# vpariza/open-hummingbird-eval

Measured on AMD Instinct MI355X. Metric: query-patches/sec, higher is better.
Workload: dtype f32

## Files before the change

### include/hbird_hip.h

```cpp
#ifndef HBIRD_HIP_H
#define HBIRD_HIP_H
#include <stdint.h>
#ifdef __cplusplus
extern "C" {
#endif

typedef struct hb_index hb_index_t;

#define HB_METRIC_IP 0
#define HB_METRIC_L2 1
#define HB_MAX_K 2048
#define HB_MAX_K_AGGREGATE 256
#define HB_BIGK_MAX_PARTS 64

const char* hb_last_error(void);
int hb_device_count(int* n);

int hb_index_create(int d, int metric, int device, hb_index_t** out);
int hb_index_free(hb_index_t* ix);
int hb_index_set_stream(hb_index_t* ix, void* hip_stream);
int hb_index_reserve(hb_index_t* ix, int64_t n_rows);
int hb_index_add(hb_index_t* ix, const float* x, int64_t n, int x_on_device, int normalize);
int hb_index_add_labels(hb_index_t* ix, const float* labels, int64_t n, int c, int on_device);
int hb_index_set_label_denominator(hb_index_t* ix, int P);
// ... 110 lines not shown
int hb_schedule_plan_weighted(int nqt, int nbt, int workgroups, int panel_tiles, int d, int cluster_q, int cluster_b, int shared,
                              const double* xcd_w8, int* segs_out, int64_t max_segs, int64_t stats[8]);
int hb_index_wg_stamps(hb_index_t* ix, uint32_t* out, int max_blocks, int* workgroups);
int hb_index_kernel_clock(hb_index_t* ix, double out[4]);
int hb_index_xcd_stats(const hb_index_t* ix, int fp16_kernel, double out[12]);
int hb_debug_live_allocations(int64_t* count, int64_t* bytes);
void* hb_calibration_new(int fp16_kernel);
void hb_calibration_free(void* h);
int hb_calibration_state(const void* h, double shares8[8], int64_t out[12]);
int hb_calibration_feed(void* h, const uint32_t* stamps, int G, const double run_shares8[8], const int key6[6], int auto_cluster, double frac);
int hb_f16_adapt_replay(int n, const double* f1, const double* f2, int64_t nq, int* out_how);
int hb_set_layout_form(int form);
int hb_index_set_rerank_copy(hb_index_t* ix, int mode);
int hb_index_rerank_copy_bytes(const hb_index_t* ix, int64_t* bytes);
int hb_index_schedule_info(const hb_index_t* ix, int64_t out[8]);
int hb_index_set_cluster(hb_index_t* ix, int cluster_q, int cluster_b, int sync_lag);
int hb_index_set_cluster_sharing(hb_index_t* ix, int mode);
int hb_index_cluster_stats(hb_index_t* ix, int64_t out[4]);

int hb_schedule_plan(int nqt, int nbt, int workgroups, int panel_tiles, int d, int cluster_q, int cluster_b, int* segs_out,
                     int64_t max_segs, int64_t stats[8]);
int hb_schedule_plan_phased(int nqt, int nbt, int workgroups, int panel_tiles, int d, int cluster_q, int cluster_b, int* segs_out,
                            int64_t max_segs, int64_t stats[8], int* clocks_out, int max_cuts, int* n_cuts, int* bounds_out);

int hb_schedule_plan_shared(int nqt, int nbt, int workgroups, int panel_tiles, int d, int cluster_q, int cluster_b, int phased,
                            int* segs_out, int64_t max_segs, int64_t stats[8]);

#include "hbird_hip_centre.h"
#include "hbird_hip_select.h"
#include "hbird_hip_grid.h"
#include "hbird_hip_exclude.h"
#include "hbird_hip_screen.h"
#include "hbird_hip_exclude_screen.h"
#include "hbird_hip_kmeans.h"
#include "hbird_hip_linprobe.h"
#include "hbird_hip_depth.h"

#ifdef __cplusplus
}
#endif
#endif
// ... 1 lines not shown
```

### open-hummingbird-eval_amd/csrc/hbird_calibrate.cpp

```cpp
#include "hbird_calibrate.h"
#include "hbird_certificate.h"
#include <algorithm>
#include <cmath>
#include <vector>

bool hb_stamps_summarise(const unsigned* st, int G, hb_stamp_summary& o) {
    if (G < 8 || G % 8 != 0) return false;
    std::vector<double> dur[8], every, ghz;
    const unsigned s0 = st[0];
    long long first = 0, last = 0;
    for (int b = 0; b < G; ++b) {
        const unsigned* sb = st + 8 * (size_t)b;
        const unsigned t0 = sb[0], t1 = sb[4], xcc = sb[1];
        if (t0 == 0u && t1 == 0u) return false;
        if (xcc > 7u || sb[5] != xcc) return false;
        if (b < 8) o.xcc[b] = (int)xcc;
        else if ((int)xcc != o.xcc[b & 7]) return false;
        const unsigned d = t1 - t0;
        if (d == 0u || d > 0x7FFFFFFFu) return false;
        dur[b & 7].push_back((double)d); every.push_back((double)d);
        const long long rs = (long long)(int)(t0 - s0), re = rs + (long long)d;
        if (b == 0) { first = rs; last = re; }
        first = std::min(first, rs); last = std::max(last, re);
        const unsigned long long c0 = ((unsigned long long)sb[3] << 32) | sb[2], c1 = ((unsigned long long)sb[7] << 32) | sb[6];
// ... 156 lines not shown
    if (in.ceil) { cq = 1; cb = 1; }
    else if (in.force_cq > 0 && in.force_cb > 0) { cq = in.force_cq; cb = in.force_cb; }
    else if (f16 && in.variant == 0 && in.force_cq == 0) {
        if (hb_stages_per_wg(nqt, nbt, G, in.dp16 / 16) >= 70000) hb_default_cluster(nqt, nbt, G, false, &cq, &cb);
    }
    else if (!f16 && !p.wide && in.variant == 0 && in.force_cq == 0 && in.g8 % 4 == 0 && hb_stages_per_wg(nqt, nbt, G, in.g8) >= 1000000) {
        p.auto_cluster = true;
        const bool measured = in.xcd_balance == 0 && G % 8 == 0;
        if (in.cl_state == 2 ? in.cl_choice != 0 : (!measured || in.cl_state == 0)) hb_default_cluster(nqt, nbt, G, true, &cq, &cb);
    }
    if ((long long)nqt * nbt < G || cq * cb > HB_CLUSTER_MAX || G % (8 * cq * cb) != 0) { cq = 1; cb = 1; }
    p.cq = cq; p.cb = cb;
    const size_t tile_bytes = (size_t)HB_BT * in.dp * 4;
    p.panel = in.force_panel > 0 ? in.force_panel : hb_default_panel(nqt, std::min<long long>(G, (long long)nqt * nbt), tile_bytes, cq, cb);
    p.phased = p.wide && in.phases_on && in.esc == 0;
    p.xs = cq * cb > 1 && (in.xcd_share == 2 || (in.xcd_share == 0 && f16));
    p.lag = cq * cb > 1 ? (in.sync_lag >= 0 ? in.sync_lag : 16) : 0;
}

void hb_knn_plan_kernel(const hb_knn_plan_in& in, int sched_G, hb_knn_plan& p) {
    const bool clustered = p.cq * p.cb > 1;
    const long long stages_per_wg = hb_stages_per_wg(p.nqt, p.nbt, sched_G, in.g8);
    p.small = !in.f16 && !clustered && stages_per_wg < (in.k > HB_KL ? std::min<long long>(p.small_limit, 50000) : p.small_limit);
    if (in.f16) p.kernel = HB_KERNEL_F16;
    else if (in.ceil) p.kernel = HB_KERNEL_CEIL;
    else if (p.bd_shape && (in.variant == 0 || in.variant == 3 || in.variant == 6)) p.kernel = HB_KERNEL_BD + (p.wide ? 4 : 0) + (clustered ? 2 : 0) + (p.small ? 1 : 0);
    else if (clustered) p.kernel = p.wide ? HB_KERNEL_POOLS_CL : HB_KERNEL_LISTS_CL;
    else if (p.small && !p.wide) p.kernel = HB_KERNEL_LISTS_COLD;
    else p.kernel = p.wide ? HB_KERNEL_POOLS : HB_KERNEL_LISTS;
}

struct hb_calibration { hb_xcd_state st; int fam; };
// ... 51 lines not shown
    hb_knn_plan_in pin;
    pin.f16 = in[0] != 0; pin.wide_first = in[1] != 0; pin.esc = (int)in[2]; pin.ceil = in[3] != 0;
    pin.k = (int)in[4]; pin.nq = in[5]; pin.ntotal = in[6]; pin.g8 = (int)in[7]; pin.dp = (int)in[8]; pin.dp16 = (int)in[9]; pin.num_cu = (int)in[10];
    pin.force_G = (int)in[11]; pin.force_panel = (int)in[12]; pin.force_cq = (int)in[13]; pin.force_cb = (int)in[14]; pin.variant = (int)in[15];
    pin.small_limit = in[16]; pin.phases_on = (int)in[17]; pin.xcd_balance = (int)in[18]; pin.xcd_share = (int)in[19]; pin.sync_lag = (int)in[20];
    pin.cl_state = (int)in[21]; pin.cl_choice = (int)in[22];
    hb_knn_plan p;
    hb_knn_plan_shape(pin, p);
    hb_knn_plan_clusters(pin, p);
    const long long pairs = (long long)p.nqt * p.nbt;
    const int sched_G = n_in > 23 && in[23] > 0 ? (int)in[23] : pairs < p.G ? (int)std::max<long long>(1, pairs) : p.G;
    hb_knn_plan_kernel(pin, sched_G, p);
    out[0] = p.kc; out[1] = p.wide; out[2] = p.klw; out[3] = p.small_pools; out[4] = p.nqt; out[5] = p.nbt; out[6] = p.G; out[7] = p.fam; out[8] = p.balance;
    out[9] = p.cq; out[10] = p.cb; out[11] = p.auto_cluster; out[12] = p.panel; out[13] = p.phased; out[14] = p.xs; out[15] = p.lag; out[16] = p.kernel;
    out[17] = sched_G; out[18] = p.small;
    return 0;
}
extern "C" int hb_certificate_bound_replay(const double* in, int n_in, double* out, int n_out) {
    if (!in || !out || n_in < 8 || n_out < 2 || !(in[0] >= 1.0 && in[0] <= 1048576.0)) return -1;
    const int d = (int)in[0], metric = in[1] != 0.0 ? 1 : 0;
    const float qn = (float)in[2], bmax = (float)in[3], qc = (float)in[4], cmax = (float)in[5], mun = (float)in[6], at = fabsf((float)in[7]);
    out[0] = (double)hb_certificate_bound(qn, bmax, d, metric);
    out[1] = (double)hb_certificate_bound_centred(qc, cmax, mun, at, qn, bmax, d, metric);
    return 0;
}
int hb_exclude_plan(int k, int64_t gmax, int rungs[2]) {
    if (k < 1 || k > HB_MAX_K || gmax < 0) return -1;
    const int64_t need = (int64_t)k + gmax;
    if (need > HB_MAX_K) return -2;
    const int64_t r0 = 256 * (((int64_t)k + std::min<int64_t>(k, gmax) + 255) / 256);
// ... 18 lines not shown
```

### open-hummingbird-eval_amd/csrc/hbird_calibrate.h

```cpp
#pragma once
#include <array>
#include <stdint.h>
#include "../../include/hbird_hip.h"
#include "hbird_schedule.h"

#define HB_POOL_MAX 512
#define HB_KL 32

struct hb_stamp_summary {
    double med[8];
    int xcc[8];
    double all;
    double span_ticks;
    double ghz_med, ghz_min, ghz_max;
};
bool hb_stamps_summarise(const unsigned* st, int G, hb_stamp_summary& o);

struct hb_xcd_state {
    double w[8] = {1, 1, 1, 1, 1, 1, 1, 1};
    int rounds = 0;
    int samples = 0, rejected = 0;
    std::array<int, 6> key{{0, 0, 0, 0, 0, 0}};
    double cur_w[8] = {1, 1, 1, 1, 1, 1, 1, 1}, best_w[8] = {1, 1, 1, 1, 1, 1, 1, 1};
    double cur_span = 0.0, best_span = 0.0;
// ... 53 lines not shown
    int phases_on = 1, xcd_balance = 0, xcd_share = 0, sync_lag = -1;
    int cl_state = 0, cl_choice = 1;
};
enum hb_knn_kernel {
    HB_KERNEL_F16 = 0,
    HB_KERNEL_LISTS = 1, HB_KERNEL_LISTS_COLD = 2, HB_KERNEL_POOLS = 3, HB_KERNEL_LISTS_CL = 4, HB_KERNEL_POOLS_CL = 5, HB_KERNEL_CEIL = 6,
    HB_KERNEL_BD = 8
};
struct hb_knn_plan {
    int kc = 0; bool wide = false; int klw = 0; bool small_pools = false;
    int nqt = 0, nbt = 0, G = 0, fam = 0; bool balance = false;
    bool calibrated = false;
    long long small_limit = 0; bool bd_shape = false;
    int cq = 1, cb = 1; bool auto_cluster = false; int panel = 0;
    bool phased = false, xs = false; int lag = 0;
    bool small = false; int kernel = HB_KERNEL_LISTS;
};
long long hb_stages_per_wg(long long nqt, long long nbt, int workgroups, int stages_per_tile);
long long hb_stages_per_busy_wg(long long nqt, long long nbt, int workgroups, int stages_per_tile);
inline int hb_knn_workgroups(int force_G, int num_cu) { return force_G > 0 ? force_G : num_cu; }
void hb_knn_plan_shape(const hb_knn_plan_in& in, hb_knn_plan& p);
void hb_knn_plan_clusters(const hb_knn_plan_in& in, hb_knn_plan& p);
void hb_knn_plan_kernel(const hb_knn_plan_in& in, int sched_G, hb_knn_plan& p);

int hb_exclude_plan(int k, int64_t gmax, int rungs[2]);
```

### open-hummingbird-eval_amd/csrc/hbird_capi.hip

```cpp
#include "../../include/hbird_hip.h"
#include "hbird_internal.h"
#include <algorithm>
#include <atomic>
#include <cmath>
#include <cstdlib>
#include <cstring>
#include <dlfcn.h>
#include <mutex>
#include <set>
#include <utility>

static thread_local std::string g_err;
void hb_set_error(const std::string& msg) { g_err = msg; }
int hb_fail(const std::string& msg) { g_err = msg; return -1; }

static std::atomic<int64_t> g_live_allocs{0}, g_live_bytes{0};
const char* hb_dev_alloc(void** p, size_t bytes) {
    const hipError_t e = hipMalloc(p, bytes);
    if (e != hipSuccess) { (void)hipGetLastError(); *p = nullptr; return hipGetErrorString(e); }
    ++g_live_allocs; g_live_bytes += (int64_t)bytes;
    return nullptr;
}
void hb_dev_free(void* p, size_t bytes) {
    (void)hipFree(p);
// ... 166 lines not shown
}
extern "C" int hb_index_last_fp16_escalated(const hb_index_t* ix, int64_t* n) {
    if (!ix || !n) return hb_fail("hb_index_last_fp16_escalated: NULL pointer");
    *n = ix->last.escalated;
    return 0;
}
extern "C" int hb_index_last_fp16_fallbacks(const hb_index_t* ix, int64_t* n) {
    if (!ix || !n) return hb_fail("hb_index_last_fp16_fallbacks: NULL pointer");
    *n = ix->last.fallbacks;
    return 0;
}


extern "C" int hb_index_set_cluster_sharing(hb_index_t* ix, int mode) {
    if (!ix) return hb_fail("hb_index_set_cluster_sharing: NULL index handle");
    if (mode < 0 || mode > 2) return hb_fail("hb_index_set_cluster_sharing: mode must be 0 (automatic), 1 (off) or 2 (on)");
    ix->xcd_share = mode; ix->sched = hb_schedule(); ix->fp32_pinned = 1;
    return 0;
}

extern "C" int hb_index_cluster_stats(hb_index_t* ix, int64_t out[4]) {
    if (!ix || !out) return hb_fail("hb_index_cluster_stats: NULL pointer");
    out[0] = out[1] = out[2] = out[3] = 0;
    if (!ix->cl_stats_dev) return 0;
    HB_HIP(hipSetDevice(ix->device));
    int h[4] = {0, 0, 0, 0};
    HB_HIP(hipMemcpyAsync(h, ix->cl_stats_dev, sizeof(h), hipMemcpyDeviceToHost, ix->stream));
    HB_HIP(hipStreamSynchronize(ix->stream));
    out[0] = h[0]; out[1] = h[1]; out[2] = h[2]; out[3] = h[3];
    return 0;
}
// ... 106 lines not shown
    }
    return 0;
}
extern "C" int hb_index_rerank_copy_bytes(const hb_index_t* ix, int64_t* bytes) {
    if (!ix || !bytes) return hb_fail("hb_index_rerank_copy_bytes: NULL argument");
    *bytes = ix->row_copy.bytes();
    return 0;
}
extern "C" int hb_index_schedule_info(const hb_index_t* ix, int64_t out[8]) {
    if (!ix) return hb_fail("hb_index_schedule_info: NULL index handle");
    const hb_schedule& s = ix->sched;
    out[0] = s.G; out[1] = (int64_t)s.segs.size(); out[2] = s.n_slots; out[3] = s.panel; out[4] = s.max_slots_per_qt;
    out[5] = s.nqt; out[6] = s.nbt; out[7] = s.cq * 16 + s.cb;
    return 0;
}

int hb_index::bank_changed(hb_bank_event what) {
    last.bank_changed();
    if (what == HB_BANK_EMPTIED) {
        copy16.emptied(); row_copy.m.emptied();
        if (copy16.flag) HB_HIP(hipMemsetAsync(copy16.flag, 0, 4, stream));
    }
    return 0;
}

extern "C" int hb_index_reserve(hb_index_t* ix, int64_t n_rows) {
    if (!ix) return hb_fail("hb_index_reserve: NULL index handle");
    HB_HIP(hipSetDevice(ix->device));
    int64_t cap = (n_rows + HB_BT - 1) / HB_BT * HB_BT;
    if (cap <= ix->cap_rows) return 0;
// ... 409 lines not shown
```

### open-hummingbird-eval_amd/csrc/hbird_knn.hip

```cpp
#include "hbird_internal.h"
#include "../../include/hbird_hip.h"
#include <algorithm>
#include <array>
#include <mutex>
#include <cstring>
#include <map>

#include "hbird_knn_dev.h"
#include "hbird_rerank_dev.h"

#define KN_MFMA(T, FR, B, S) acc[T] = __builtin_amdgcn_mfma_f32_32x32x2f32(FR[(T) & 3][S], B[S], acc[T], 0, 0, 0);

template <bool COLD, bool WIDE, bool CL = false, bool CEIL = false>
__global__ __launch_bounds__(HB_THREADS, 2) void knn_fused_kernel(knn_args a) {
    extern __shared__ __attribute__((aligned(16))) char smem[];
    const int tid = threadIdx.x;
    const int lane = tid & 63;
    const int w = __builtin_amdgcn_readfirstlane(tid >> 6);
    const int h = lane >> 5;
    float* lst_s = reinterpret_cast<float*>(smem + KN_LISTS);
    unsigned* lst_i = reinterpret_cast<unsigned*>(smem + KN_LISTS + HB_QT * HB_KL * 4);
    float* sc = reinterpret_cast<float*>(smem + KN_SCRATCH) + w * 256;
    unsigned* qf = reinterpret_cast<unsigned*>(smem + KN_QF) + w * 512;
    int* pcnt = reinterpret_cast<int*>(smem + KN_LISTS);
// ... 596 lines not shown
    knn_work_list& wl = *out;
    static const double equal_shares[8] = {1, 1, 1, 1, 1, 1, 1, 1};
    if (p.balance) {
        double shares_n[8];
        double mean = 0.0;
        bool uneven = false;
        const hb_index::xcd_cal& xc = ix->xcal[p.fam];
        for (int x = 0; x < 8; ++x) mean += xc.w[x] / 8.0;
        for (int g = 0; g < 8; ++g) { shares_n[g] = xc.w[ix->xcd_balance == 0 ? xc.perm[g] : g] / mean; uneven = uneven || std::fabs(shares_n[g] - 1.0) > 1e-9; }
        if (uneven) std::copy(shares_n, shares_n + 8, wl.shares);
    }
    const double* shares = wl.shares;
    hb_schedule& sc = esc == 0 ? ix->sched : ix->sched_esc;
    hb_dev<char>& sched_dev = esc == 0 ? ix->sched_dev : ix->sched_esc_dev;
    const int nqt = p.nqt, nbt = p.nbt, G = p.G;
    const bool rebuilt = !(sc.nqt == nqt && sc.nbt == nbt && sc.panel == p.panel && sc.cq == p.cq && sc.cb == p.cb && sc.phased == p.phased &&
                           sc.xcd_share == p.xs && (sc.G == G || (long long)nqt * nbt < G) &&
                           (sc.xcd_w.empty() ? std::equal(shares, shares + 8, equal_shares) : std::equal(shares, shares + 8, sc.xcd_w.begin())));
    if (rebuilt) { hb_build_schedule(nqt, nbt, G, p.panel, sc, p.cq, p.cb, p.phased, p.xs, shares); ++ix->sched_builds; }
    const struct { const void* data; size_t bytes; } part[6] = {{sc.segs.data(), sc.segs.size() * sizeof(hb_seg)}, {sc.wg_off.data(), sc.wg_off.size() * 4},
        {sc.qt_off.data(), sc.qt_off.size() * 4}, {sc.qt_slots.data(), sc.qt_slots.size() * 4}, {sc.wg_member.data(), sc.wg_member.size() * 4},
        {sc.phase_bounds.data(), sc.phase_bounds.size() * 4}};
    size_t off[7] = {0};
    for (int i = 0; i < 6; ++i) off[i + 1] = off[i] + al256(part[i].bytes);
    const bool need_upload = rebuilt || sched_dev.bytes < off[6];
    if (sched_dev.ensure(off[6], HB_GROW_QUARTER)) return -1;
    if (need_upload) {
        for (int i = 0; i < 6; ++i) HB_HIP(hipMemcpyAsync(sched_dev + off[i], part[i].data, part[i].bytes, hipMemcpyHostToDevice, s));
        HB_HIP(hipStreamSynchronize(s));
    }
    auto ints = [&](int i) { return sched_dev.as<const int>(off[i]); };
    wl.sc = &sc; wl.segs = sched_dev.as<const hb_seg>();
    wl.wg_off = ints(1); wl.qt_off = ints(2); wl.qt_slots = ints(3); wl.wg_member = ints(4); wl.phase_bounds = ints(5);
    wl.n_phases = (int)sc.phase_clock.size() + 1;
// ... 326 lines not shown
```

### open-hummingbird-eval_amd/csrc/hbird_schedule.cpp

```cpp
#include "hbird_schedule.h"
#include <algorithm>
#include <cmath>
#include <map>

#ifdef HB_PLAN_STANDALONE
static thread_local std::string g_plan_err;
int hb_fail(const std::string& msg) { g_plan_err = msg; return -1; }
extern "C" const char* hb_last_error(void) { return g_plan_err.c_str(); }
#endif

static int hb_gcd(int x, int y) { while (y) { int t = x % y; x = y; y = t; } return x; }

int hb_default_panel(int nqt, int G, size_t tile_bytes, int cq, int cb) {
    int p0;
    if (cq * cb > 1) {
        const int NC = std::max(1, G / (cq * cb)), NQG = (nqt + cq - 1) / cq;
        p0 = cb * (NC / hb_gcd(NQG, NC));
    } else p0 = G / hb_gcd(nqt, G);
    size_t budget = (size_t)96 << 20;
    int j = (int)std::max<size_t>(1, budget / (tile_bytes * (size_t)p0));
    return p0 * j;
}

void hb_default_cluster(int nqt, int nbt, int G, bool fp32_kernel, int* cq, int* cb) {
// ... 82 lines not shown
}

static std::vector<double> hb_cum_shares(int workers, int per_xcd, const std::vector<double>& xcd_w) {
    std::vector<double> cum(workers + 1, 0.0);
    for (int i = 0; i < workers; ++i) cum[i + 1] = cum[i] + xcd_w[std::min(7, i / std::max(1, per_xcd))];
    for (int i = 0; i <= workers; ++i) cum[i] /= cum[workers];
    return cum;
}
static long long hb_share_bound(long long W, const std::vector<double>& cum, int i, int workers, int panel_index) {
    if (i <= 0) return 0;
    if (i >= workers) return W;
    const double phi = std::fmod(0.5 + 0.6180339887498949 * panel_index, 1.0);
    return std::min<long long>(W, std::max<long long>(0, (long long)std::floor((double)W * cum[i] + phi)));
}

static void hb_build_clustered(int nqt, int nbt, int G, int panel, int cq, int cb, hb_schedule& out, bool xcd_share) {
    const int CS = cq * cb, NC = G / CS, NQG = (nqt + cq - 1) / cq;
    out.cq = cq; out.cb = cb; out.n_clusters = NC; out.xcd_share = xcd_share;
    std::vector<std::vector<hb_seg>> per_wg(G);
    std::vector<int> slot_of((size_t)G * nqt, -1);
    std::vector<std::vector<int>> slots_of_qt(nqt);
    std::vector<int> clock(NC, 0);
    auto deal = [&](int c, int b0, int pp, int qg, int j0, int cnt) {
        for (int m = 0; m < CS; ++m) {
            const int ia = m / cb, ib = m % cb, q = qg * cq + ia, w = c * CS + m;
            int n = cnt;
            if ((j0 + cnt - 1) * cb + ib >= pp) --n;
            if (q >= nqt || n <= 0) continue;
            hb_seg sg;
            sg.q_tile = q; sg.b_tile0 = b0 + j0 * cb + ib; sg.n_tiles = n; sg.stride = cb; sg.tile0 = clock[c]; sg.next_tile0 = 0;
            int& known = slot_of[(size_t)w * nqt + q];
            if (known < 0) {
                sg.slot = out.n_slots++; sg.first = 1;
                known = sg.slot;
                slots_of_qt[q].push_back(sg.slot);
            } else { sg.slot = known; sg.first = 0; }
            per_wg[w].push_back(sg);
        }
        clock[c] += cnt;
    };
    const int per_xcd_c = NC / 8;
    int rot = 0;
    const std::vector<double> cum = (!out.xcd_w.empty() && !xcd_share && NC % 8 == 0) ? hb_cum_shares(NC, NC / 8, out.xcd_w) : std::vector<double>();
    const std::vector<double> cumx = (!out.xcd_w.empty() && xcd_share) ? hb_cum_shares(8, 1, out.xcd_w) : std::vector<double>();
    for (int b0 = 0; b0 < nbt; b0 += panel) {
        const int pp = std::min(panel, nbt - b0);
        const int UB = (pp + cb - 1) / cb;
        const long long U = (long long)NQG * UB;
        if (xcd_share) {
            for (int x = 0; x < 8; ++x) {
                long long e = (U * x) / 8;
                long long e1 = (U * (x + 1)) / 8;
                if (!cumx.empty()) { e = hb_share_bound(U, cumx, x, 8, b0 / panel); e1 = hb_share_bound(U, cumx, x + 1, 8, b0 / panel); }
                while (e < e1) {
                    const int qg = (int)(e / UB), j0 = (int)(e % UB);
                    const int L = (int)std::min<long long>(UB - j0, e1 - e);
                    for (int i = 0; i < per_xcd_c; ++i) {
                        const int a0 = (int)((long long)L * i / per_xcd_c), a1 = (int)((long long)L * (i + 1) / per_xcd_c);
                        if (a1 > a0) deal(x * per_xcd_c + (i + rot) % per_xcd_c, b0, pp, qg, j0 + a0, a1 - a0);
                    }
                    ++rot;
                    e += L;
                }
            }
            continue;
        }
        for (int c = 0; c < NC; ++c) {
            long long e0 = (U * c) / NC, e1 = (U * (c + 1)) / NC;
            if (!cum.empty()) { e0 = hb_share_bound(U, cum, c, NC, b0 / panel); e1 = hb_share_bound(U, cum, c + 1, NC, b0 / panel); }
            while (e0 < e1) {
                const int qg = (int)(e0 / UB), j0 = (int)(e0 % UB);
                const int cnt = (int)std::min<long long>(UB - j0, e1 - e0);
                deal(c, b0, pp, qg, j0, cnt);
                e0 += cnt;
            }
        }
    }
    std::vector<int> logical_of_block(G);
    out.wg_member.assign(G, -1);
    const int per_xcd = NC / 8;
    for (int c = 0; c < NC; ++c)
        for (int m = 0; m < CS; ++m) {
            const int block = c / per_xcd + 8 * ((c % per_xcd) * CS + m);
            logical_of_block[block] = c * CS + m;
            out.wg_member[block] = c * HB_CLUSTER_LINE + m;
        }
    hb_finish_schedule(out, per_wg, logical_of_block, slots_of_qt);
}

void hb_build_schedule(int nqt, int nbt, int G, int panel, hb_schedule& out, int cq, int cb, bool phased, bool xcd_share, const double* xcd_w) {
    out = hb_schedule();
    out.nqt = nqt; out.nbt = nbt; out.panel = panel; out.phased = phased;
    if (xcd_w) {
        bool ok = true, equal = true;
        for (int x = 0; x < 8; ++x) { ok = ok && xcd_w[x] > 0.25 && xcd_w[x] < 4.0; equal = equal && xcd_w[x] == xcd_w[0]; }
        if (ok && !equal) out.xcd_w.assign(xcd_w, xcd_w + 8);
    }
    const long long total_pairs = (long long)nqt * nbt;
    if (total_pairs < G) G = (int)std::max<long long>(1, total_pairs);
    out.G = G;
    if (phased) {
        const long long per_wg_tiles = total_pairs / G;
        long long t = 0, step = 1;
        while (out.phase_clock.size() < HB_PHASE_CUTS) {
            t += step;
            if (t * 2 > per_wg_tiles) break;
            out.phase_clock.push_back((int)t);
            step = std::max<long long>(step + 1, per_wg_tiles <= 64 ? step * 3 : step < 128 ? step * 3 / 2 : step * 2);
        }
    }
    if (cq < 1 || cb < 1 || cq * cb > HB_CLUSTER_MAX || G % (8 * cq * cb) != 0) { cq = 1; cb = 1; }
    if (cq * cb > 1) { hb_build_clustered(nqt, nbt, G, panel, cq, cb, out, xcd_share); return; }
    std::vector<std::vector<hb_seg>> per_wg(G);
    std::vector<int> slot_of((size_t)G * nqt, -1);
    std::vector<std::vector<int>> slots_of_qt(nqt);
    std::vector<int> clock(G, 0);
    const std::vector<double> cum = (!out.xcd_w.empty() && G % 8 == 0) ? hb_cum_shares(G, G / 8, out.xcd_w) : std::vector<double>();
    for (int b0 = 0; b0 < nbt; b0 += panel) {
        const int pp = std::min(panel, nbt - b0);
        const long long W = (long long)nqt * pp;
        for (int w = 0; w < G; ++w) {
            long long e0 = (W * w) / G, e1 = (W * (w + 1)) / G;
            if (!cum.empty()) { e0 = hb_share_bound(W, cum, w, G, b0 / panel); e1 = hb_share_bound(W, cum, w + 1, G, b0 / panel); }
            while (e0 < e1) {
                const int q = (int)(e0 / pp), b = (int)(e0 % pp);
                const int cnt = (int)std::min<long long>(pp - b, e1 - e0);
                int& known = slot_of[(size_t)w * nqt + q];
// ... 16 lines not shown
    }
    std::vector<int> logical_of_block(G);
    for (int b = 0; b < G; ++b) {
        if (G % 8 == 0) logical_of_block[b] = (b % 8) * (G / 8) + b / 8;
        else {
            const int q = G / 8, r = G % 8, x = b % 8;
            logical_of_block[b] = (x < r ? x * (q + 1) : r * (q + 1) + (x - r) * q) + b / 8;
        }
    }
    out.wg_member.assign(G, -1);
    hb_finish_schedule(out, per_wg, logical_of_block, slots_of_qt);
}


static int schedule_plan(int nqt, int nbt, int workgroups, int panel_tiles, int d, int cluster_q, int cluster_b, bool phased,
                         int* segs_out, int64_t max_segs, int64_t stats[8], hb_schedule& sc, bool xcd_share = false, const double* xcd_w = nullptr) {
    if (!stats) return hb_fail("hb_schedule_plan: stats is NULL");
    if (nqt <= 0 || nbt <= 0 || workgroups <= 0 || d <= 0) return hb_fail("hb_schedule_plan: bad arguments");
    const int dp = (d + HB_KC - 1) / HB_KC * HB_KC;
    const int G = (int)std::min<long long>(workgroups, (long long)nqt * nbt);
    int cq = cluster_q, cb = cluster_b;
    if (cq < 0 || cb < 0) hb_default_cluster(nqt, nbt, G, cq == -2, &cq, &cb);
    if (cq < 1 || cb < 1 || (long long)nqt * nbt < workgroups || cq * cb > HB_CLUSTER_MAX || G % (8 * cq * cb) != 0) { cq = 1; cb = 1; }
    const int panel = panel_tiles > 0 ? panel_tiles : hb_default_panel(nqt, G, (size_t)HB_BT * dp * 4, cq, cb);
    hb_build_schedule(nqt, nbt, workgroups, panel, sc, cq, cb, phased, xcd_share && cq * cb > 1, xcd_w);
    stats[0] = sc.G; stats[1] = (int64_t)sc.segs.size(); stats[2] = sc.n_slots; stats[3] = sc.panel;
    stats[4] = sc.max_slots_per_qt; stats[5] = sc.nqt; stats[6] = sc.nbt; stats[7] = sc.cq * 16 + sc.cb;
    if (segs_out) {
        int64_t n = 0;
        for (int b = 0; b < sc.G; ++b)
            for (int i = sc.wg_off[b]; i < sc.wg_off[b + 1] && n < max_segs; ++i, ++n) {
                const hb_seg& g = sc.segs[i];
                int* o = segs_out + n * 10;
                o[0] = b; o[1] = g.q_tile; o[2] = g.b_tile0; o[3] = g.n_tiles; o[4] = g.slot; o[5] = g.first;
                o[6] = g.stride; o[7] = g.tile0; o[8] = g.next_tile0; o[9] = sc.wg_member[b];
            }
    }
    return 0;
}

// ... 17 lines not shown
    }
    return 0;
}

extern "C" int hb_schedule_plan_weighted(int nqt, int nbt, int workgroups, int panel_tiles, int d, int cluster_q, int cluster_b, int shared,
                                         const double* xcd_w8, int* segs_out, int64_t max_segs, int64_t stats[8]) {
    hb_schedule sc;
    return schedule_plan(nqt, nbt, workgroups, panel_tiles, d, cluster_q, cluster_b, (shared & 2) != 0, segs_out, max_segs, stats, sc, (shared & 1) != 0, xcd_w8);
}

extern "C" int hb_schedule_plan_shared(int nqt, int nbt, int workgroups, int panel_tiles, int d, int cluster_q, int cluster_b, int phased,
                                       int* segs_out, int64_t max_segs, int64_t stats[8]) {
    hb_schedule sc;
    return schedule_plan(nqt, nbt, workgroups, panel_tiles, d, cluster_q, cluster_b, phased != 0, segs_out, max_segs, stats, sc, true);
}
```

### open-hummingbird-eval_amd/csrc/hbird_schedule.h

```cpp
#pragma once
#include <stddef.h>
#include <stdint.h>
#include <string>
#include <vector>

#define HB_QT 256
#define HB_BT 256
#define HB_KC 16

struct hb_seg {
    int q_tile;
    int b_tile0;
    int n_tiles;
    int slot;
    int first;
    int stride;
    int tile0;
    int next_tile0;
    int ord;
    int nsl;
};

#define HB_PHASE_CUTS 24
#define HB_CLUSTER_MAX 8
// ... 4 lines not shown
    int cq = 1, cb = 1;
    bool xcd_share = false;
    std::vector<double> xcd_w;
    std::vector<hb_seg> segs;
    std::vector<int> wg_off;
    std::vector<int> wg_member;
    bool phased = false;
    std::vector<int> phase_clock;
    bool cuts_scaled = false;
    std::vector<int> phase_bounds;
    std::vector<int> qt_off;
    std::vector<int> qt_slots;
    int n_slots = 0;
    int max_slots_per_qt = 0;
    int n_clusters = 0;
};

void hb_build_schedule(int nqt, int nbt, int G, int panel_tiles, hb_schedule& out, int cq = 1, int cb = 1, bool phased = false,
                       bool xcd_share = false, const double* xcd_w = nullptr);
int hb_default_panel(int nqt, int G, size_t tile_bytes, int cq = 1, int cb = 1);
void hb_default_cluster(int nqt, int nbt, int G, bool fp32_kernel, int* cq, int* cb);

int hb_fail(const std::string& msg);
```

### open-hummingbird-eval_amd/hbird_mi/_lib.py

```python
from __future__ import annotations

import ctypes
import os
from ctypes import POINTER, c_char_p, c_double, c_float, c_int, c_int32, c_int64, c_uint64, c_void_p

_PKG_ROOT = os.path.dirname(os.path.dirname(os.path.abspath(__file__)))
LIB_PATH = os.environ.get("HBIRD_HIP_LIB") or os.path.join(_PKG_ROOT, "lib", "libhbird_hip.so")
CSRC_DIR = os.path.join(_PKG_ROOT, "csrc")

_lib = None

SIGNATURES = {
    "hb_last_error": (c_char_p, []),
    "hb_device_count": (c_int, [POINTER(c_int)]),
    "hb_index_create": (c_int, [c_int, c_int, c_int, POINTER(c_void_p)]),
    "hb_index_free": (c_int, [c_void_p]),
    "hb_index_set_stream": (c_int, [c_void_p, c_void_p]),
    "hb_index_reserve": (c_int, [c_void_p, c_int64]),
    "hb_index_add": (c_int, [c_void_p, c_void_p, c_int64, c_int, c_int]),
    "hb_index_add_labels": (c_int, [c_void_p, c_void_p, c_int64, c_int, c_int]),
    "hb_index_ntotal": (c_int64, [c_void_p]),
    "hb_index_nlabels": (c_int64, [c_void_p]),
    "hb_index_reset": (c_int, [c_void_p]),
    "hb_index_search": (c_int, [c_void_p, c_void_p, c_int64, c_int, c_int64, c_void_p, c_void_p, c_int]),
# ... 41 lines not shown
                                       c_void_p]),
    "hb_argmax_channels": (c_int, [c_void_p, c_int64, c_int, c_void_p, c_void_p]),
    "hb_confusion_update": (c_int, [c_void_p, c_void_p, c_int64, c_int, c_int, c_int64, c_int, c_void_p, c_void_p]),
    "hb_index_set_timing": (c_int, [c_void_p, c_int]),
    "hb_index_last_knn_ms": (c_int, [c_void_p, POINTER(c_double)]),
    "hb_index_set_tuning": (c_int, [c_void_p, c_int, c_int]),
    "hb_index_set_fp16": (c_int, [c_void_p, c_int]),
    "hb_index_last_fp16_fallbacks": (c_int, [c_void_p, POINTER(c_int64)]),
    "hb_last_search_path": (c_int, [c_void_p, POINTER(c_int), POINTER(c_int)]),
    "hb_index_set_fp16_escalation": (c_int, [c_void_p, c_int]),
    "hb_index_last_fp16_escalated": (c_int, [c_void_p, POINTER(c_int64)]),
    "hb_schedule_plan": (c_int, [c_int, c_int, c_int, c_int, c_int, c_int, c_int, c_void_p, c_int64, POINTER(c_int64)]),
    "hb_schedule_plan_phased": (c_int, [c_int, c_int, c_int, c_int, c_int, c_int, c_int, c_void_p, c_int64, POINTER(c_int64),
                                        c_void_p, c_int, POINTER(c_int), c_void_p]),
    "hb_schedule_plan_shared": (c_int, [c_int, c_int, c_int, c_int, c_int, c_int, c_int, c_int, c_void_p, c_int64, POINTER(c_int64)]),
    "hb_index_set_cluster": (c_int, [c_void_p, c_int, c_int, c_int]),
    "hb_index_set_cluster_sharing": (c_int, [c_void_p, c_int]),
    "hb_index_set_label_denominator": (c_int, [c_void_p, c_int]),
    "hb_index_labels_to_fp32": (c_int, [c_void_p]),
    "hb_index_label_denominator": (c_int, [c_void_p, POINTER(c_int)]),
    "hb_index_copy_label_counts": (c_int, [c_void_p, c_void_p, c_int]),
    "hb_index_set_label_count_table": (c_int, [c_void_p, c_void_p, c_void_p, c_int64, c_int, c_int, c_int64]),
    "hb_index_cluster_stats": (c_int, [c_void_p, POINTER(c_int64)]),
    "hb_index_set_variant": (c_int, [c_void_p, c_int]),
    "hb_index_set_search_options": (c_int, [c_void_p, c_int, c_int64]),
    "hb_index_wg_stamps": (c_int, [c_void_p, c_void_p, c_int, POINTER(c_int)]),
    "hb_index_set_xcd_weights": (c_int, [c_void_p, c_int, POINTER(c_double)]),
    "hb_index_xcd_weights": (c_int, [c_void_p, c_int, POINTER(c_double), POINTER(c_int)]),
    "hb_schedule_plan_weighted": (c_int, [c_int, c_int, c_int, c_int, c_int, c_int, c_int, c_int, POINTER(c_double), c_void_p, c_int64, POINTER(c_int64)]),
    "hb_index_kernel_clock": (c_int, [c_void_p, POINTER(c_double)]),
# ... 172 lines not shown
```

### open-hummingbird-eval_amd/hbird_mi/nn/search_hip.py

```python
from __future__ import annotations

import ctypes
import math
from collections import namedtuple
from typing import Optional, Tuple

import numpy as np
import torch

from hbird_mi import _lib
from hbird_mi.nn.search_base import NearestNeighborSearchBase

_METRICS = {"dot_product": 0, "l2": 1, "euclidean": 1}
MAX_K = 256
MAX_K_SEARCH = 2048
_MERGE_LDS = 60000


def k5(index, name: str, k: int):
    return getattr(index, name + "_bigk" if k > MAX_K and hasattr(index, name + "_bigk") else name)


def check_k(k: int, what: str = "k"):
    if not 1 <= k <= MAX_K_SEARCH:
# ... 615 lines not shown

    def set_cluster_sharing(self, mode: int = 0):
        _lib.check(_lib.lib().hb_index_set_cluster_sharing(self._h, int(mode)))

    def cluster_stats(self) -> dict:
        out = (ctypes.c_int64 * 4)()
        _lib.check(_lib.lib().hb_index_cluster_stats(self._h, out))
        return {"checks": int(out[0]), "waits": int(out[1]), "timeouts": int(out[2])}

    def schedule_info(self) -> dict:
        out = (ctypes.c_int64 * 8)()
        _lib.check(_lib.lib().hb_index_schedule_info(self._h, out))
        keys = ["workgroups", "segments", "slots", "panel_tiles", "max_slots_per_qtile", "query_tiles", "bank_tiles"]
        d = dict(zip(keys, list(out)[:7]))
        d["cluster"] = [int(out[7]) // 16, int(out[7]) % 16]
        return d


def _merge_fits_lds(parts: int, k: int) -> bool:
    n = parts * k
    return (n * 4 + 15) // 16 * 16 + n * 8 <= _MERGE_LDS


def merge_topk(dist_parts: torch.Tensor, idx_parts: torch.Tensor, metric: int):
    parts, nq, k = dist_parts.shape
    dist_parts = dist_parts.contiguous(); idx_parts = idx_parts.contiguous()
    idx = torch.empty((nq, k), dtype=torch.int64, device=dist_parts.device)
    dist = torch.empty((nq, k), dtype=torch.float32, device=dist_parts.device)
    s = torch.cuda.current_stream(dist_parts.device).cuda_stream
    entry = _lib.lib().hb_merge_topk if _merge_fits_lds(parts, k) else _lib.lib().hb_bigk_merge_topk
# ... 498 lines not shown
```

Before: 81320.

## Fill leftover query-tile rows in clustered schedule with narrower, wider-bank units

When the query-tile count is not a multiple of the cluster height, the clustered schedule previously dealt a full cq-tall unit for the remainder, leaving some cluster members idle. The new 'filled' mode splits the remainder into power-of-two sub-rows whose bank width is widened (CS/part), so every member of a cluster works. It is on by default for the fp16 clustered path, with a fallback to the old schedule when slots per query tile would exceed an LDS-derived limit. It also adds idle-tick accounting and introspection APIs.

```diff
diff --git a/include/hbird_hip.h b/include/hbird_hip.h
--- a/include/hbird_hip.h
+++ b/include/hbird_hip.h
@@ -148,6 +148,7 @@
 int hb_index_set_rerank_copy(hb_index_t* ix, int mode);
 int hb_index_rerank_copy_bytes(const hb_index_t* ix, int64_t* bytes);
 int hb_index_schedule_info(const hb_index_t* ix, int64_t out[8]);
+int hb_last_schedule_fill(const hb_index_t* ix, int64_t out[4]);
 int hb_index_set_cluster(hb_index_t* ix, int cluster_q, int cluster_b, int sync_lag);
 int hb_index_set_cluster_sharing(hb_index_t* ix, int mode);
 int hb_index_cluster_stats(hb_index_t* ix, int64_t out[4]);
@@ -159,6 +160,9 @@
 
 int hb_schedule_plan_shared(int nqt, int nbt, int workgroups, int panel_tiles, int d, int cluster_q, int cluster_b, int phased,
                             int* segs_out, int64_t max_segs, int64_t stats[8]);
+int hb_schedule_plan_filled(int nqt, int nbt, int workgroups, int panel_tiles, int d, int cluster_q, int cluster_b, int phased, int xcd_share,
+                            const double* xcd_w8, int slot_limit, int* segs_out, int64_t max_segs, int64_t stats[12], int* clocks_out,
+                            int max_cuts, int* n_cuts, int* bounds_out);
 
 #include "hbird_hip_centre.h"
 #include "hbird_hip_select.h"
diff --git a/open-hummingbird-eval_amd/csrc/hbird_calibrate.cpp b/open-hummingbird-eval_amd/csrc/hbird_calibrate.cpp
--- a/open-hummingbird-eval_amd/csrc/hbird_calibrate.cpp
+++ b/open-hummingbird-eval_amd/csrc/hbird_calibrate.cpp
@@ -194,8 +194,17 @@
     const size_t tile_bytes = (size_t)HB_BT * in.dp * 4;
     p.panel = in.force_panel > 0 ? in.force_panel : hb_default_panel(nqt, std::min<long long>(G, (long long)nqt * nbt), tile_bytes, cq, cb);
     p.phased = p.wide && in.phases_on && in.esc == 0;
-    p.xs = cq * cb > 1 && (in.xcd_share == 2 || (in.xcd_share == 0 && f16));
+    p.xs = cq * cb > 1 && (in.xcd_share >= 2 || (in.xcd_share == 0 && f16));
+    p.filled = f16 && cq * cb > 1 && nqt > cq && nqt % cq != 0 && (in.xcd_share == 3 || in.xcd_share == 0);
     p.lag = cq * cb > 1 ? (in.sync_lag >= 0 ? in.sync_lag : 16) : 0;
+}
+
+int hb_fill_slot_limit(int klw, int kc, bool phased) {
+    const long long lds = 48 * 1024 / 8;
+    const long long w = std::max(1, klw), k = std::max(1, kc);
+    long long lim = lds / w >= 2 ? std::max<long long>(lds / w, (lds / w) * (lds / k)) : 2 * (lds / k);
+    if (phased) lim = std::min<long long>(lim, 144 * 1024 / 16 / w);
+    return (int)std::max<long long>(1, std::min<long long>(lim, 1 << 20));
 }
 
 void hb_knn_plan_kernel(const hb_knn_plan_in& in, int sched_G, hb_knn_plan& p) {
@@ -277,6 +286,7 @@
     out[0] = p.kc; out[1] = p.wide; out[2] = p.klw; out[3] = p.small_pools; out[4] = p.nqt; out[5] = p.nbt; out[6] = p.G; out[7] = p.fam; out[8] = p.balance;
     out[9] = p.cq; out[10] = p.cb; out[11] = p.auto_cluster; out[12] = p.panel; out[13] = p.phased; out[14] = p.xs; out[15] = p.lag; out[16] = p.kernel;
     out[17] = sched_G; out[18] = p.small;
+    if (n_out > 19) out[19] = p.filled;
     return 0;
 }
 extern "C" int hb_certificate_bound_replay(const double* in, int n_in, double* out, int n_out) {
diff --git a/open-hummingbird-eval_amd/csrc/hbird_calibrate.h b/open-hummingbird-eval_amd/csrc/hbird_calibrate.h
--- a/open-hummingbird-eval_amd/csrc/hbird_calibrate.h
+++ b/open-hummingbird-eval_amd/csrc/hbird_calibrate.h
@@ -91,6 +91,7 @@
     long long small_limit = 0; bool bd_shape = false;
     int cq = 1, cb = 1; bool auto_cluster = false; int panel = 0;
     bool phased = false, xs = false; int lag = 0;
+    bool filled = false;
     bool small = false; int kernel = HB_KERNEL_LISTS;
 };
 long long hb_stages_per_wg(long long nqt, long long nbt, int workgroups, int stages_per_tile);
@@ -99,5 +100,6 @@
 void hb_knn_plan_shape(const hb_knn_plan_in& in, hb_knn_plan& p);
 void hb_knn_plan_clusters(const hb_knn_plan_in& in, hb_knn_plan& p);
 void hb_knn_plan_kernel(const hb_knn_plan_in& in, int sched_G, hb_knn_plan& p);
+int hb_fill_slot_limit(int klw, int kc, bool phased);
 
 int hb_exclude_plan(int k, int64_t gmax, int rungs[2]);
diff --git a/open-hummingbird-eval_amd/csrc/hbird_capi.hip b/open-hummingbird-eval_amd/csrc/hbird_capi.hip
--- a/open-hummingbird-eval_amd/csrc/hbird_capi.hip
+++ b/open-hummingbird-eval_amd/csrc/hbird_capi.hip
@@ -204,7 +204,7 @@
 
 extern "C" int hb_index_set_cluster_sharing(hb_index_t* ix, int mode) {
     if (!ix) return hb_fail("hb_index_set_cluster_sharing: NULL index handle");
-    if (mode < 0 || mode > 2) return hb_fail("hb_index_set_cluster_sharing: mode must be 0 (automatic), 1 (off) or 2 (on)");
+    if (mode < 0 || mode > 3) return hb_fail("hb_index_set_cluster_sharing: mode must be 0 (automatic), 1 (off), 2 (on) or 3 (on, filled)");
     ix->xcd_share = mode; ix->sched = hb_schedule(); ix->fp32_pinned = 1;
     return 0;
 }
@@ -341,6 +341,12 @@
     out[5] = s.nqt; out[6] = s.nbt; out[7] = s.cq * 16 + s.cb;
     return 0;
 }
+extern "C" int hb_last_schedule_fill(const hb_index_t* ix, int64_t out[4]) {
+    if (!ix || !out) return hb_fail("hb_last_schedule_fill: NULL argument");
+    const hb_schedule& s = ix->sched;
+    out[0] = s.filled; out[1] = s.idle_member_ticks; out[2] = s.member_ticks; out[3] = s.fill_refused;
+    return 0;
+}
 
 int hb_index::bank_changed(hb_bank_event what) {
     last.bank_changed();
diff --git a/open-hummingbird-eval_amd/csrc/hbird_knn.hip b/open-hummingbird-eval_amd/csrc/hbird_knn.hip
--- a/open-hummingbird-eval_amd/csrc/hbird_knn.hip
+++ b/open-hummingbird-eval_amd/csrc/hbird_knn.hip
@@ -634,10 +634,11 @@
     hb_schedule& sc = esc == 0 ? ix->sched : ix->sched_esc;
     hb_dev<char>& sched_dev = esc == 0 ? ix->sched_dev : ix->sched_esc_dev;
     const int nqt = p.nqt, nbt = p.nbt, G = p.G;
+    const int fill_limit = p.filled ? hb_fill_slot_limit(p.klw, p.kc, p.phased) : 0;
     const bool rebuilt = !(sc.nqt == nqt && sc.nbt == nbt && sc.panel == p.panel && sc.cq == p.cq && sc.cb == p.cb && sc.phased == p.phased &&
-                           sc.xcd_share == p.xs && (sc.G == G || (long long)nqt * nbt < G) &&
+                           sc.xcd_share == p.xs && sc.fill_asked == p.filled && sc.fill_slot_limit == fill_limit && (sc.G == G || (long long)nqt * nbt < G) &&
                            (sc.xcd_w.empty() ? std::equal(shares, shares + 8, equal_shares) : std::equal(shares, shares + 8, sc.xcd_w.begin())));
-    if (rebuilt) { hb_build_schedule(nqt, nbt, G, p.panel, sc, p.cq, p.cb, p.phased, p.xs, shares); ++ix->sched_builds; }
+    if (rebuilt) { hb_build_schedule(nqt, nbt, G, p.panel, sc, p.cq, p.cb, p.phased, p.xs, shares, p.filled, fill_limit); ++ix->sched_builds; }
     const struct { const void* data; size_t bytes; } part[6] = {{sc.segs.data(), sc.segs.size() * sizeof(hb_seg)}, {sc.wg_off.data(), sc.wg_off.size() * 4},
         {sc.qt_off.data(), sc.qt_off.size() * 4}, {sc.qt_slots.data(), sc.qt_slots.size() * 4}, {sc.wg_member.data(), sc.wg_member.size() * 4},
         {sc.phase_bounds.data(), sc.phase_bounds.size() * 4}};
diff --git a/open-hummingbird-eval_amd/csrc/hbird_schedule.cpp b/open-hummingbird-eval_amd/csrc/hbird_schedule.cpp
--- a/open-hummingbird-eval_amd/csrc/hbird_schedule.cpp
+++ b/open-hummingbird-eval_amd/csrc/hbird_schedule.cpp
@@ -120,21 +120,35 @@
     return std::min<long long>(W, std::max<long long>(0, (long long)std::floor((double)W * cum[i] + phi)));
 }
 
-static void hb_build_clustered(int nqt, int nbt, int G, int panel, int cq, int cb, hb_schedule& out, bool xcd_share) {
-    const int CS = cq * cb, NC = G / CS, NQG = (nqt + cq - 1) / cq;
+struct hb_unit_row { int q0, qw, bw; };
+
+static void hb_build_clustered(int nqt, int nbt, int G, int panel, int cq, int cb, hb_schedule& out, bool xcd_share, bool filled) {
+    const int CS = cq * cb, NC = G / CS;
     out.cq = cq; out.cb = cb; out.n_clusters = NC; out.xcd_share = xcd_share;
+    std::vector<hb_unit_row> rows;
+    for (int q = 0; q + cq <= nqt; q += cq) rows.push_back({q, cq, cb});
+    const int q_left = nqt / cq * cq, r = nqt - q_left;
+    filled = filled && r > 0 && nqt >= cq && (cq & (cq - 1)) == 0;
+    out.filled = filled;
+    if (r > 0 && !filled) rows.push_back({q_left, cq, cb});
+    if (filled)
+        for (int part = cq >> 1, q = q_left; part >= 1; part >>= 1)
+            if (r & part) { rows.push_back({q, part, CS / part}); q += part; }
+    const int NR = (int)rows.size();
     std::vector<std::vector<hb_seg>> per_wg(G);
     std::vector<int> slot_of((size_t)G * nqt, -1);
     std::vector<std::vector<int>> slots_of_qt(nqt);
     std::vector<int> clock(NC, 0);
-    auto deal = [&](int c, int b0, int pp, int qg, int j0, int cnt) {
+    auto deal = [&](int c, int b0, int pp, const hb_unit_row& rw, int j0, int cnt) {
         for (int m = 0; m < CS; ++m) {
-            const int ia = m / cb, ib = m % cb, q = qg * cq + ia, w = c * CS + m;
+            const int ia = m / rw.bw, ib = m % rw.bw, q = rw.q0 + ia, w = c * CS + m;
             int n = cnt;
-            if ((j0 + cnt - 1) * cb + ib >= pp) --n;
-            if (q >= nqt || n <= 0) continue;
+            if ((j0 + cnt - 1) * rw.bw + ib >= pp) --n;
+            out.member_ticks += cnt;
+            if (q >= nqt || n <= 0) { out.idle_member_ticks += cnt; continue; }
+            out.idle_member_ticks += cnt - n;
             hb_seg sg;
-            sg.q_tile = q; sg.b_tile0 = b0 + j0 * cb + ib; sg.n_tiles = n; sg.stride = cb; sg.tile0 = clock[c]; sg.next_tile0 = 0;
+            sg.q_tile = q; sg.b_tile0 = b0 + j0 * rw.bw + ib; sg.n_tiles = n; sg.stride = rw.bw; sg.tile0 = clock[c]; sg.next_tile0 = 0;
             int& known = slot_of[(size_t)w * nqt + q];
             if (known < 0) {
                 sg.slot = out.n_slots++; sg.first = 1;
@@ -149,21 +163,28 @@
     int rot = 0;
     const std::vector<double> cum = (!out.xcd_w.empty() && !xcd_share && NC % 8 == 0) ? hb_cum_shares(NC, NC / 8, out.xcd_w) : std::vector<double>();
     const std::vector<double> cumx = (!out.xcd_w.empty() && xcd_share) ? hb_cum_shares(8, 1, out.xcd_w) : std::vector<double>();
+    std::vector<long long> first(NR + 1, 0);
     for (int b0 = 0; b0 < nbt; b0 += panel) {
         const int pp = std::min(panel, nbt - b0);
-        const int UB = (pp + cb - 1) / cb;
-        const long long U = (long long)NQG * UB;
+        for (int i = 0; i < NR; ++i) first[i + 1] = first[i] + (pp + rows[i].bw - 1) / rows[i].bw;
+        const long long U = first[NR];
+        auto run_at = [&](long long e, long long e1, int* j0, int* len) {
+            const int i = (int)(std::upper_bound(first.begin(), first.end(), e) - first.begin()) - 1;
+            *j0 = (int)(e - first[i]);
+            *len = (int)std::min<long long>(first[i + 1] - e, e1 - e);
+            return i;
+        };
         if (xcd_share) {
             for (int x = 0; x < 8; ++x) {
                 long long e = (U * x) / 8;
                 long long e1 = (U * (x + 1)) / 8;
                 if (!cumx.empty()) { e = hb_share_bound(U, cumx, x, 8, b0 / panel); e1 = hb_share_bound(U, cumx, x + 1, 8, b0 / panel); }
                 while (e < e1) {
-                    const int qg = (int)(e / UB), j0 = (int)(e % UB);
-                    const int L = (int)std::min<long long>(UB - j0, e1 - e);
-                    for (int i = 0; i < per_xcd_c; ++i) {
-                        const int a0 = (int)((long long)L * i / per_xcd_c), a1 = (int)((long long)L * (i + 1) / per_xcd_c);
-                        if (a1 > a0) deal(x * per_xcd_c + (i + rot) % per_xcd_c, b0, pp, qg, j0 + a0, a1 - a0);
+                    int j0, L;
+                    const int i = run_at(e, e1, &j0, &L);
+                    for (int ci = 0; ci < per_xcd_c; ++ci) {
+                        const int a0 = (int)((long long)L * ci / per_xcd_c), a1 = (int)((long long)L * (ci + 1) / per_xcd_c);
+                        if (a1 > a0) deal(x * per_xcd_c + (ci + rot) % per_xcd_c, b0, pp, rows[i], j0 + a0, a1 - a0);
                     }
                     ++rot;
                     e += L;
@@ -175,9 +196,9 @@
             long long e0 = (U * c) / NC, e1 = (U * (c + 1)) / NC;
             if (!cum.empty()) { e0 = hb_share_bound(U, cum, c, NC, b0 / panel); e1 = hb_share_bound(U, cum, c + 1, NC, b0 / panel); }
             while (e0 < e1) {
-                const int qg = (int)(e0 / UB), j0 = (int)(e0 % UB);
-                const int cnt = (int)std::min<long long>(UB - j0, e1 - e0);
-                deal(c, b0, pp, qg, j0, cnt);
+                int j0, cnt;
+                const int i = run_at(e0, e1, &j0, &cnt);
+                deal(c, b0, pp, rows[i], j0, cnt);
                 e0 += cnt;
             }
         }
@@ -194,7 +215,19 @@
     hb_finish_schedule(out, per_wg, logical_of_block, slots_of_qt);
 }
 
-void hb_build_schedule(int nqt, int nbt, int G, int panel, hb_schedule& out, int cq, int cb, bool phased, bool xcd_share, const double* xcd_w) {
+static void hb_build_schedule_as(int nqt, int nbt, int G, int panel, hb_schedule& out, int cq, int cb, bool phased, bool xcd_share, const double* xcd_w,
+                                 bool filled);
+
+void hb_build_schedule(int nqt, int nbt, int G, int panel, hb_schedule& out, int cq, int cb, bool phased, bool xcd_share, const double* xcd_w, bool filled,
+                       int fill_slot_limit) {
+    hb_build_schedule_as(nqt, nbt, G, panel, out, cq, cb, phased, xcd_share, xcd_w, filled);
+    const bool refused = out.filled && fill_slot_limit > 0 && out.max_slots_per_qt > fill_slot_limit;
+    if (refused) hb_build_schedule_as(nqt, nbt, G, panel, out, cq, cb, phased, xcd_share, xcd_w, false);
+    out.fill_asked = filled; out.fill_slot_limit = fill_slot_limit; out.fill_refused = refused;
+}
+
+static void hb_build_schedule_as(int nqt, int nbt, int G, int panel, hb_schedule& out, int cq, int cb, bool phased, bool xcd_share, const double* xcd_w,
+                                 bool filled) {
     out = hb_schedule();
     out.nqt = nqt; out.nbt = nbt; out.panel = panel; out.phased = phased;
     if (xcd_w) {
@@ -216,7 +249,7 @@
         }
     }
     if (cq < 1 || cb < 1 || cq * cb > HB_CLUSTER_MAX || G % (8 * cq * cb) != 0) { cq = 1; cb = 1; }
-    if (cq * cb > 1) { hb_build_clustered(nqt, nbt, G, panel, cq, cb, out, xcd_share); return; }
+    if (cq * cb > 1) { hb_build_clustered(nqt, nbt, G, panel, cq, cb, out, xcd_share, filled); return; }
     std::vector<std::vector<hb_seg>> per_wg(G);
     std::vector<int> slot_of((size_t)G * nqt, -1);
     std::vector<std::vector<int>> slots_of_qt(nqt);
@@ -263,7 +296,8 @@
 
 
 static int schedule_plan(int nqt, int nbt, int workgroups, int panel_tiles, int d, int cluster_q, int cluster_b, bool phased,
-                         int* segs_out, int64_t max_segs, int64_t stats[8], hb_schedule& sc, bool xcd_share = false, const double* xcd_w = nullptr) {
+                         int* segs_out, int64_t max_segs, int64_t stats[8], hb_schedule& sc, bool xcd_share = false, const double* xcd_w = nullptr,
+                         bool filled = false, int fill_slot_limit = 0) {
     if (!stats) return hb_fail("hb_schedule_plan: stats is NULL");
     if (nqt <= 0 || nbt <= 0 || workgroups <= 0 || d <= 0) return hb_fail("hb_schedule_plan: bad arguments");
     const int dp = (d + HB_KC - 1) / HB_KC * HB_KC;
@@ -272,7 +306,7 @@
     if (cq < 0 || cb < 0) hb_default_cluster(nqt, nbt, G, cq == -2, &cq, &cb);
     if (cq < 1 || cb < 1 || (long long)nqt * nbt < workgroups || cq * cb > HB_CLUSTER_MAX || G % (8 * cq * cb) != 0) { cq = 1; cb = 1; }
     const int panel = panel_tiles > 0 ? panel_tiles : hb_default_panel(nqt, G, (size_t)HB_BT * dp * 4, cq, cb);
-    hb_build_schedule(nqt, nbt, workgroups, panel, sc, cq, cb, phased, xcd_share && cq * cb > 1, xcd_w);
+    hb_build_schedule(nqt, nbt, workgroups, panel, sc, cq, cb, phased, xcd_share && cq * cb > 1, xcd_w, filled && cq * cb > 1, fill_slot_limit);
     stats[0] = sc.G; stats[1] = (int64_t)sc.segs.size(); stats[2] = sc.n_slots; stats[3] = sc.panel;
     stats[4] = sc.max_slots_per_qt; stats[5] = sc.nqt; stats[6] = sc.nbt; stats[7] = sc.cq * 16 + sc.cb;
     if (segs_out) {
@@ -320,3 +354,20 @@
     hb_schedule sc;
     return schedule_plan(nqt, nbt, workgroups, panel_tiles, d, cluster_q, cluster_b, phased != 0, segs_out, max_segs, stats, sc, true);
 }
+
+extern "C" int hb_schedule_plan_filled(int nqt, int nbt, int workgroups, int panel_tiles, int d, int cluster_q, int cluster_b, int phased, int xcd_share,
+                                       const double* xcd_w8, int slot_limit, int* segs_out, int64_t max_segs, int64_t stats[12], int* clocks_out,
+                                       int max_cuts, int* n_cuts, int* bounds_out) {
+    if (slot_limit < 0) return hb_fail("hb_schedule_plan_filled: bad slot limit");
+    hb_schedule sc;
+    if (schedule_plan(nqt, nbt, workgroups, panel_tiles, d, cluster_q, cluster_b, phased != 0, segs_out, max_segs, stats, sc, xcd_share != 0, xcd_w8, true,
+                      slot_limit)) return -1;
+    stats[8] = sc.filled; stats[9] = sc.idle_member_ticks; stats[10] = sc.member_ticks; stats[11] = sc.fill_refused;
+    if (n_cuts) *n_cuts = (int)sc.phase_clock.size();
+    for (int p = 0; p < (int)sc.phase_clock.size() && p < max_cuts; ++p) {
+        if (clocks_out) clocks_out[p] = sc.phase_clock[p];
+        if (bounds_out)
+            for (int b = 0; b < sc.G; ++b) bounds_out[(size_t)p * sc.G + b] = sc.phase_bounds[(size_t)p * sc.G + b] - sc.wg_off[b];
+    }
+    return 0;
+}
diff --git a/open-hummingbird-eval_amd/csrc/hbird_schedule.h b/open-hummingbird-eval_amd/csrc/hbird_schedule.h
--- a/open-hummingbird-eval_amd/csrc/hbird_schedule.h
+++ b/open-hummingbird-eval_amd/csrc/hbird_schedule.h
@@ -42,10 +42,16 @@
     int n_slots = 0;
     int max_slots_per_qt = 0;
     int n_clusters = 0;
+    bool fill_asked = false;
+    int fill_slot_limit = 0;
+    bool filled = false;
+    bool fill_refused = false;
+    long long member_ticks = 0;
+    long long idle_member_ticks = 0;
 };
 
 void hb_build_schedule(int nqt, int nbt, int G, int panel_tiles, hb_schedule& out, int cq = 1, int cb = 1, bool phased = false,
-                       bool xcd_share = false, const double* xcd_w = nullptr);
+                       bool xcd_share = false, const double* xcd_w = nullptr, bool filled = false, int fill_slot_limit = 0);
 int hb_default_panel(int nqt, int G, size_t tile_bytes, int cq = 1, int cb = 1);
 void hb_default_cluster(int nqt, int nbt, int G, bool fp32_kernel, int* cq, int* cb);
 
diff --git a/open-hummingbird-eval_amd/hbird_mi/_lib.py b/open-hummingbird-eval_amd/hbird_mi/_lib.py
--- a/open-hummingbird-eval_amd/hbird_mi/_lib.py
+++ b/open-hummingbird-eval_amd/hbird_mi/_lib.py
@@ -79,6 +79,9 @@
     "hb_schedule_plan_phased": (c_int, [c_int, c_int, c_int, c_int, c_int, c_int, c_int, c_void_p, c_int64, POINTER(c_int64),
                                         c_void_p, c_int, POINTER(c_int), c_void_p]),
     "hb_schedule_plan_shared": (c_int, [c_int, c_int, c_int, c_int, c_int, c_int, c_int, c_int, c_void_p, c_int64, POINTER(c_int64)]),
+    "hb_schedule_plan_filled": (c_int, [c_int, c_int, c_int, c_int, c_int, c_int, c_int, c_int, c_int, c_void_p, c_int, c_void_p, c_int64,
+                                        POINTER(c_int64), c_void_p, c_int, POINTER(c_int), c_void_p]),
+    "hb_last_schedule_fill": (c_int, [c_void_p, POINTER(c_int64)]),
     "hb_index_set_cluster": (c_int, [c_void_p, c_int, c_int, c_int]),
     "hb_index_set_cluster_sharing": (c_int, [c_void_p, c_int]),
     "hb_index_set_label_denominator": (c_int, [c_void_p, c_int]),
diff --git a/open-hummingbird-eval_amd/hbird_mi/nn/search_hip.py b/open-hummingbird-eval_amd/hbird_mi/nn/search_hip.py
--- a/open-hummingbird-eval_amd/hbird_mi/nn/search_hip.py
+++ b/open-hummingbird-eval_amd/hbird_mi/nn/search_hip.py
@@ -653,6 +653,11 @@
         keys = ["workgroups", "segments", "slots", "panel_tiles", "max_slots_per_qtile", "query_tiles", "bank_tiles"]
         d = dict(zip(keys, list(out)[:7]))
         d["cluster"] = [int(out[7]) // 16, int(out[7]) % 16]
+        fill = (ctypes.c_int64 * 4)()
+        _lib.check(_lib.lib().hb_last_schedule_fill(self._h, fill))
+        d["filled"] = int(fill[0]); d["idle_member_ticks"] = int(fill[1]); d["member_ticks"] = int(fill[2])
+        if fill[3]:
+            d["fill_refused"] = 1
         return d
 
 
```

Measured after the change: 83220 (median of 6 runs). 1.02x the previous value.
